# MeirBon/rendering-fw

Hardware: AMD Instinct MI355X
Metric: Msamples/sec at 1920x1080, 1M-tri scene; 1/2/4/8-GPU tile scaling (higher is better)
Workload: dtype f32; 1 GPU; terrain_1002k: 1002536 triangles, 1920x1080, pt integrator depth 2, 256 spp per step, 8 area-light triangles + 2 point lights, synthetic 2048x1024 HDR sky; parallelism=single GPU, no collective, streams=4, sample_group=64, csrc_hash=108fd956ff29d79e

## Files before the change

rendering-fw_amd/csrc/kernels.h:

```cpp
#pragma once
#include "rt_types.h"
#include <stddef.h>

namespace rtk
{

struct Params
{
	rt::SceneView sc;
	rt::WaveView wv;
	rt::CamView cam;
	rt::FrameView fr;
	uint32_t depth;
	uint32_t max_depth;
	uint32_t parity_no_jitter;
	uint32_t lds_first;
	uint32_t lds_count;
	uint32_t queue;
	uint32_t group;
	uint32_t refill;
	uint32_t textured;
};

enum GenMode
{
	GEN_BUFFER = 0,
	GEN_PT = 1,
	GEN_PARITY = 2,
	GEN_RANGED = 3
};

typedef void *stream_t;

struct DnView
{
	uint32_t W, H;
	rt::f4 *ga, *gb;
	rt::f4 *in, *out;
	rt::f4 *img[2];
	float *var[2];
	float sigma_l, sigma_n, sigma_z;
	uint32_t iterations;
	uint32_t *overflow;
	uint32_t *id;
	rt::f4 *hist;
};

struct DnTemporal
{
	rt::CamView cam, pcam;
	rt::FrameView fr;
	const rt::f4 *pgb;
	const uint32_t *id, *pid;
	const uint32_t *inst_ver;
	uint32_t n_inst, pscene;
	const rt::f4 *col_in;
	const float *mom_in, *n_in;
	float *mom_out, *n_out;
	float alpha;
	uint32_t usable;
};

constexpr uint32_t DN_M_INVALID = 0u, DN_M_STILL = 1u, DN_M_MOVED = 2u, DN_M_RESTART = 3u;
struct alignas(16) DnMotionInst
{
	float mp[12], mf[12];
	const rt::f4 *cur, *prev;
	const uint32_t *indices;
	uint32_t state, tri_count, vert_count, pad;
};
struct DnMotion
{
	const DnMotionInst *inst;
	const rt::f4 *surf;
// ... 117 lines not shown
```

rendering-fw_amd/csrc/kernels.hip:

```cpp
#include "kernels.h"
#include "rt_core.h"
#include "emu_streams.h"

#include <string.h>
#include <algorithm>

using namespace rt;

namespace rtk
{

constexpr int BLOCK = 256;
constexpr int KAT_IN = 24, KAT_OUT = 8;
#ifndef RT_TRAVERSAL_WAVES
#define RT_TRAVERSAL_WAVES 6
#endif
#ifndef RT_TRACE_WAVES
#define RT_TRACE_WAVES 8
#endif
#ifndef RT_TRACE_VGPRS
#define RT_TRACE_VGPRS 64
#endif
#ifndef RT_PRIMARY_WAVES
#define RT_PRIMARY_WAVES 7
// ... 65 lines not shown
	Ctx() { stk.lds = lds, stk.spill = spill, pot = potbuf, stk.top = nullptr, stk.top_first = 0, stk.top_count = 0, stk.overflow = &overflow_sink, stk.stride = 1; }
	explicit Ctx(const Params &p) : Ctx()
	{
		stk.overflow = &p.wv.counters->stack_overflow;
		stk.top = (const f4 *)(p.sc.nodes4 + p.lds_first), stk.top_first = p.lds_first, stk.top_count = p.lds_count;
	}
	struct OutQueue
	{
		uint32_t rays = 0;
	};
	OutQueue q_ext, q_shadow;
	uint32_t alloc(OutQueue &q, bool flag, uint32_t *queue_len)
	{
		if (!flag)
			return 0u;
		q.rays++;
		return (*queue_len)++;
	}
	void add64(unsigned long long *dst, uint32_t v) { *dst += v; }
};

#endif

RT_FN void primary_finish_item(const Params &q, uint32_t idx, f3 D, const Hit &h)
{
	int prim = h.prim;
	if (prim < 0)
	{
		f3 radiance = mk3(0, 0, 0);
		const f3 contribution = (mk3(1, 1, 1) * m_rcp(1.0f)) * pt_sky(q.sc, D);
		if (!any_nan(contribution))
			radiance = clamp_intensity(contribution, q.cam.clamp_value);
		q.wv.rad[idx] = mk4(radiance.x, radiance.y, radiance.z, q.wv.rad_nee ? -1.0f : 1.0f);
		prim = HIT_MISS_SHADED;
	}
	q.wv.hit0[idx] = mk4(h.t, h.u, h.v, ubits((uint32_t)prim));
	q.wv.hit0_inst[idx] = h.inst;
	if (prim >= 0)
	{
		float zero = 0.0f, one = 1.0f;
#if defined(__HIP_DEVICE_COMPILE__)
		asm volatile("" : "+v"(zero), "+v"(one));
#endif
		q.wv.rad[idx] = mk4(zero, zero, zero, one);
	}
}

template <int GEN, bool COUNT>
RT_FN void extend_item(const Params &p, uint32_t i, bool active, Ctx &ctx)
{
	f3 O = mk3(0, 0, 0), D = mk3(0, 0, 1);
	const uint32_t b = p.depth & 1u;
	float t_min = 1e-5f, t_max = 1e34f;
	if (GEN == GEN_BUFFER || GEN == GEN_RANGED)
	{
		if (active)
		{
			const f4 o4 = p.wv.org[b][i], d4 = p.wv.dir[b][i];
			O = xyz(o4), D = xyz(d4);
			if (GEN == GEN_RANGED)
				t_min = o4.w, t_max = d4.w;
			else if (fbits(o4.w) == RAY_VOID)
			{
				p.wv.hit[i] = mk4(0, 0, 0, ubits((uint32_t)HIT_VOID));
				active = false;
			}
		}
	}
	else
	{
		const PixelRef pr = slot_to_pixel(p.fr, i);
		active = active && pr.valid;
		if (GEN == GEN_PT)
		{
			if (active)
				pt_primary_ray(p.cam, p.fr, pr.x, pr.y, p.fr.sample_base + pr.sample, O, D);
		}
		else
		{
			const uint32_t npx = p.fr.W / 4u, npy = p.fr.H / 2u;
			active = active && pr.x < npx * 4u && pr.y < npy * 2u;
			if (active)
			{
				float r0 = 0.5f, r1 = 0.5f, r2 = 0.5f, r3 = 0.5f;
				if (!p.parity_no_jitter)
				{
					const uint32_t packet = (pr.y / 2u) * npx + pr.x / 4u;
					const uint32_t lane = (pr.y & 1u) * 4u + (pr.x & 3u);
					const uint32_t *sp = p.wv.packet_rng + 4ull * ((unsigned long long)pr.sample * npx * npy + packet);
					uint32_t s[4] = {sp[0], sp[1], sp[2], sp[3]};
					const bool lens = p.cam.aperture != 0.0f;
					const uint32_t draws = lens ? 32u : 16u;
					for (uint32_t k = 0; k < draws; k++)
					{
						const float r = u32_to_unit(xor128_next(s));
						if (k == lane)
							r0 = r;
						else if (k == 8u + lane)
							r1 = r;
						else if (k == 16u + lane)
							r2 = r;
						else if (k == 24u + lane)
							r3 = r;
					}
				}
				parity_primary_ray(p.cam, p.fr, pr.x, pr.y, r0, r1, r2, r3, O, D);
			}
		}
		if (active && GEN != GEN_PT)
		{
			p.wv.org[0][i] = mk4(O.x, O.y, O.z, ubits((i << 1) | 1u));
			p.wv.dir[0][i] = mk4(D.x, D.y, D.z, 0.0f);
		}
	}
	Hit h;
	h.t = 1e34f, h.u = 0, h.v = 0, h.prim = -1, h.inst = -1;
	TStat st;
	st.inner = 0, st.tris = 0, st.lds = 0;
	if (active)
	{
		trace<false, COUNT>(p.sc, O, D, t_min, t_max, h, ctx.stk, st);
		if (GEN == GEN_PT)
			primary_finish_item(p, i, D, h);
		else
		{
			f4 *hb = p.depth == 0 ? p.wv.hit0 : p.wv.hit;
			int *ib = p.depth == 0 ? p.wv.hit0_inst : p.wv.hit_inst;
			hb[i] = mk4(h.t, h.u, h.v, ubits((uint32_t)h.prim));
			ib[i] = h.inst;
		}
	}
	if (COUNT)
	{
		ctx.add64(&p.wv.counters->inner_extend, st.inner);
		ctx.add64(&p.wv.counters->tris_extend, st.tris);
		ctx.add64(&p.wv.counters->lds_extend, st.lds);
		ctx.add64(&p.wv.counters->rays_extend, active ? 1u : 0u);
	}
}

template <bool COUNT>
RT_FN void shade_parity_item(const Params &p, uint32_t i, bool active, Ctx &ctx)
{
	const PixelRef pr = slot_to_pixel(p.fr, i);
	active = active && pr.valid && pr.x < (p.fr.W / 4u) * 4u && pr.y < (p.fr.H / 2u) * 2u;
	TStat st;
	st.inner = 0, st.tris = 0, st.lds = 0;
	uint32_t nshadow = 0;
	f4 out = mk4(0, 0, 0, 0);
	if (active)
	{
		const f4 o4 = p.wv.org[0][i], d4 = p.wv.dir[0][i], h4 = p.wv.hit0[i];
		Hit h;
		h.t = h4.x, h.u = h4.y, h.v = h4.z, h.prim = (int)fbits(h4.w), h.inst = p.wv.hit0_inst[i];
		if (h.prim < 0)
		{
			const f3 s = parity_sky(p.sc, xyz(d4));
			out = mk4(s.x, s.y, s.z, 0.0f);
		}
		else
		{
			if (pr.sample == 0 && pr.y * p.fr.W + pr.x == p.fr.probe_pixel)
			{
				WaveCounters *c = p.wv.counters;
				c->probe_inst = (uint32_t)h.inst, c->probe_prim = (uint32_t)h.prim, c->probe_dist = h.t, c->probe_valid = 1u;
			}
			out = parity_shade<COUNT>(p.sc, xyz(o4), xyz(d4), h, ctx.stk, st, nshadow);
		}
	}
	if (pr.valid)
		p.wv.rad[i] = out;
	if (COUNT)
	{
		ctx.add64(&p.wv.counters->inner_shadow, st.inner);
		ctx.add64(&p.wv.counters->tris_shadow, st.tris);
		ctx.add64(&p.wv.counters->lds_shadow, st.lds);
		ctx.add64(&p.wv.counters->rays_shadow, nshadow);
		ctx.add64(&p.wv.counters->shaded, (active && out.w > 0.0f) ? 1u : 0u);
	}
}

#if defined(RT_DIAG_SHADE_CLOCK)
__device__ unsigned long long g_shade_clk[32];
#define RT_ITEM_CLK , ClkProbe *clk
#define RT_ITEM_TICK(K) clk_tick(*clk, K)
#else
#define RT_ITEM_CLK
#define RT_ITEM_TICK(K)
#endif
struct ShadeSink
{
	const Params &p;
	Ctx &ctx;
	uint32_t slot;
	RT_FN void probe(const Hit &h) const
	{
		WaveCounters *c = p.wv.counters;
		c->probe_inst = (uint32_t)h.inst, c->probe_prim = (uint32_t)h.prim, c->probe_dist = h.t, c->probe_valid = 1u;
	}
	RT_FN void shadow(bool emit, const f4 &so, const f4 &sd, const f4 &se)
	{
		const uint32_t si = ctx.alloc(ctx.q_shadow, emit, &p.wv.counters->shadow_n[p.depth]);
		if (emit)
		{
			p.wv.sh_org[si] = so;
			p.wv.sh_dir[si] = sd;
			if (p.depth != 0 || !p.wv.rad_nee)
				p.wv.sh_rad[si] = se;
			else
				p.wv.rad_nee[slot] = mk4(0.0f + se.x, 0.0f + se.y, 0.0f + se.z, 0.0f);
		}
	}
};

template <bool TEX, bool SKY, bool LT> RT_FN void shade_pt_item(const Params &p, const SkyView &sky, const LightTreeView &lt, uint32_t i, bool active, const f4 &h4, int hi, Ctx &ctx RT_ITEM_CLK)
{
	RT_ITEM_TICK(0);
	const uint32_t b = p.depth & 1u, nb = b ^ 1u;
	ShadeOut out;
	PathIn in;
	in.O = mk3(0, 0, 0), in.D = mk3(0, 0, 1), in.T = mk3(1, 1, 1), in.bsdfPdf = 1.0f;
	in.slot = 0, in.flags = 0, in.packedN = 0, in.depth = p.depth;
	Hit h;
	h.t = h4.x, h.u = h4.y, h.v = h4.z, h.prim = (int)fbits(h4.w), h.inst = hi;
	if (active && p.depth == 0)
	{
		const PixelRef pr = slot_to_pixel(p.fr, i);
		pt_primary_ray(p.cam, p.fr, pr.x, pr.y, p.fr.sample_base + pr.sample, in.O, in.D);
		in.slot = i, in.flags = 1u, in.packedN = 0u;
	}
	else if (active)
	{
		const f4 o4 = (p.depth == 0 && p.cam.aperture == 0.0f) ? mk4(p.cam.pos.x, p.cam.pos.y, p.cam.pos.z, ubits((i << 1) | 1u)) : p.wv.org[b][i];
		const f4 d4 = p.wv.dir[b][i];
		in.O = xyz(o4), in.D = xyz(d4);
		const uint32_t ow = fbits(o4.w);
		in.slot = ow >> 1, in.flags = ow & 1u, in.packedN = fbits(d4.w);
		if (p.depth != 0)
		{
			const f4 t4 = p.wv.thr[b][i];
			in.T = xyz(t4), in.bsdfPdf = t4.w;
		}
	}
	const uint32_t slot = in.slot;
	ShadeSink sink{p, ctx, slot};
	pt_shade<TEX, SKY, LT>(p.sc, sky, lt, p.cam, p.fr, p.max_depth, active, in, h, out, ctx.pot, sink RT_CLK_ARG);
	if (active)
	{
		if (p.depth == 0)
		{
			const bool ends = p.wv.rad_nee && !out.emit_shadow && !out.emit_ext;
			if (h.prim < 0 || ends || out.radiance.x != 0.0f || out.radiance.y != 0.0f || out.radiance.z != 0.0f)
				p.wv.rad[slot] = mk4(out.radiance.x, out.radiance.y, out.radiance.z, ends ? -1.0f : 1.0f);
			if (p.wv.rad_nee && out.emit_ext && !out.emit_shadow)
				p.wv.rad_nee[slot] = mk4(0, 0, 0, 0);
		}
		else if (out.radiance.x != 0.0f || out.radiance.y != 0.0f || out.radiance.z != 0.0f)
		{
			f4 r = p.wv.rad[slot];
			r.x += out.radiance.x, r.y += out.radiance.y, r.z += out.radiance.z;
			p.wv.rad[slot] = r;
		}
	}
	RT_ITEM_TICK(7);
	const uint32_t ei = ctx.alloc(ctx.q_ext, out.emit_ext, &p.wv.counters->ext_n[p.depth + 1]);
	if (out.emit_ext)
	{
		p.wv.org[nb][ei] = out.eo;
		p.wv.dir[nb][ei] = out.ed;
		p.wv.thr[nb][ei] = out.et;
	}
	RT_ITEM_TICK(8);
}

RT_FN void connect_finish(const Params &p, uint32_t i, uint32_t slot, bool visible)
{
	if (p.depth == 0 && p.wv.rad_nee)
	{
		if (!visible)
			p.wv.rad_nee[slot] = mk4(0, 0, 0, 0);
	}
	else if (visible)
	{
		const f4 e4 = p.wv.sh_rad[i];
		f4 *const dst = p.wv.rad_nee ? p.wv.rad_nee : p.wv.rad;
		f4 r = dst[slot];
		r.x += e4.x, r.y += e4.y, r.z += e4.z;
		dst[slot] = r;
	}
}
RT_FN uint32_t shadow_slot(const Params &p, uint32_t word)
{
	return (p.depth == 0 && p.fr.shadow_bins) ? word & ((1u << shadow_slot_bits(p.fr.shadow_bins)) - 1u) : word;
}
RT_FN void connect_skip_item(const Params &p, uint32_t i)
// ... 655 lines not shown
			const uint32_t base = q_next;
			const uint32_t take = nidle < q_end - q_next ? nidle : q_end - q_next;
			q_next += take;
			const uint32_t limit = base + take;
			if (!has_ray)
			{
				const uint32_t idx = base + wave_prefix(idle_mask);
				if (idx < limit)
				{
					{
						typedef float v4f_ __attribute__((ext_vector_type(4)));
						v4f_ oa = *(const v4f_ *)(ray_o + idx), da = *(const v4f_ *)(ray_d + idx);
						asm volatile("" : "+v"(oa), "+v"(da));
						const f4 o4 = mk4(oa.x, oa.y, oa.z, oa.w), d4 = mk4(da.x, da.y, da.z, da.w);
						if (fbits(o4.w) == RAY_VOID)
						{
							if (!ANY)
								p.wv.hit[idx] = mk4(0, 0, 0, ubits((uint32_t)HIT_VOID));
						}
						else
						{
							T.begin(p.sc, xyz(o4), xyz(d4), 1e-5f, ANY ? d4.w : 1e34f);
							has_ray = true, ray = idx, slot = ANY ? shadow_slot(p, fbits(o4.w)) : fbits(o4.w), nrays++;
						}
					}
				}
			}
			exhausted = q_next >= count;
		}
		if (__ballot(has_ray) == 0ull)
		{
			if (exhausted)
				break;
			continue;
		}
		RT_TRACE_TICK(0)
		T.template descend<VOTE>(p.sc, ctx.stk, st);
		RT_TRACE_TICK(1)
		const auto world = [&](f3 &O, f3 &D) {
			const f4 o4 = ray_o[ray], d4 = ray_d[ray];
			O = xyz(o4), D = xyz(d4);
		};
		if (has_ray)
			T.visit(p.sc, ctx.stk, st, world);
		RT_TRACE_TICK(2)
		if (has_ray)
		{
			if (T.done())
			{
				if (ANY)
					connect_finish(p, ray, slot, T.hit.prim < 0);
				else
				{
					p.wv.hit[ray] = mk4(T.hit.t, T.hit.u, T.hit.v, ubits((uint32_t)T.hit.prim));
					p.wv.hit_inst[ray] = T.hit.inst;
				}
				has_ray = false;
			}
		}
		RT_TRACE_TICK(3)
	}
#if defined(RT_DIAG_TRACE_CLOCK)
	if (lane == 0u)
		for (int k = 0; k < 4; k++)
			atomicAdd(&g_trace_clk[MODE == STREAM_ANY ? 1 : 0][k], clk_acc[k]), atomicAdd(&g_trace_clk[MODE == STREAM_ANY ? 1 : 0][4 + k], clk_n[k]);
#endif
	if (COUNT)
	{
		ctx.add64(ANY ? &wc->inner_shadow : &wc->inner_extend, st.inner);
		ctx.add64(ANY ? &wc->tris_shadow : &wc->tris_extend, st.tris);
		ctx.add64(ANY ? &wc->lds_shadow : &wc->lds_extend, st.lds);
		ctx.add64(ANY ? &wc->rays_shadow : &wc->rays_extend, nrays);
	}
}

template <bool ANY, bool COUNT>
__global__ void __launch_bounds__(TRACE_BLOCK, ANY ? RT_ANY_WAVES : RT_TRACE_WAVES) __attribute__((amdgpu_num_vgpr(RT_TRACE_VGPRS))) k_trace_stream(const Params p)
{
	const uint32_t count = ANY ? connection_count(p.wv.counters, p.depth) : p.wv.counters->ext_n[p.depth];
	if (count == 0u)
	{
		if (ANY && p.depth == 0 && p.wv.rad_nee)
			for (uint32_t i = blockIdx.x * TRACE_BLOCK + threadIdx.x, n = p.wv.counters->shadow_n[0]; i < n; i += gridDim.x * TRACE_BLOCK)
				connect_skip_item(p, i);
		return;
	}
	if (!ANY)
		clock_in(p.wv.counters, p.depth);
	RT_STACK_DECL_N(ANY ? LDS_STACK_ANY : LDS_STACK, TRACE_BLOCK)
	stream_rays<ANY ? STREAM_ANY : STREAM_EXT, COUNT>(p, count, ctx);
	if (!ANY)
		clock_out(p.wv.counters, p.depth);
}

template <bool COUNT>
__global__ void __launch_bounds__(TRACE_BLOCK, RT_TRACE_WAVES) __attribute__((amdgpu_num_vgpr(RT_TRACE_VGPRS))) k_trace_fused(const Params pe, const Params pa)
{
	const uint32_t count_e = pe.wv.counters->ext_n[pe.depth];
	const uint32_t count_a = connection_count(pa.wv.counters, pa.depth);
	if (count_a == 0u && pa.depth == 0 && pa.wv.rad_nee)
		for (uint32_t i = blockIdx.x * TRACE_BLOCK + threadIdx.x, n = pa.wv.counters->shadow_n[0]; i < n; i += gridDim.x * TRACE_BLOCK)
			connect_skip_item(pa, i);
	if (count_e == 0u && count_a == 0u)
		return;
	const Params &p = pe;
	RT_STACK_DECL_N(LDS_STACK, TRACE_BLOCK)
	const unsigned long long t0 = threadIdx.x == 0 ? (unsigned long long)wall_clock64() : 0ull;
	if (count_e)
// ... 1214 lines not shown
```

rendering-fw_amd/csrc/rfwhip_api.cpp:

```cpp
#include "rfwhip.h"

#include "bvh_build.h"
#include "device_layer.h"
#include "internal.h"
#include "kernels.h"
#include "rt_types.h"
#include "sky_sampling.h"
#include "light_tree.h"

#include <algorithm>
#include <chrono>
#include <cmath>
#include <cstdarg>
#include <cstdio>
#include <cstdlib>
#include <cstring>
#include <string>
#include <vector>

using rt::f4;

static thread_local char g_error[1024] = "";
int rfwhip_internal_set_error(int code, const char *fmt, ...)
{
// ... 237 lines not shown
	int dn_temporal = 0;
	float dn_alpha = 0.2f;
	DevBuf d_dn_prev, d_dn_ids, d_dn_hist, d_dn_inst_ver;
	unsigned long long frame_serial = 0;
	unsigned long long samples_total = 0;
	uint32_t sample_origin = 0;
	bool dn_have_pres = false;
	unsigned long long dn_pres_serial = 0;
	rt::CamView dn_pres_cam{};
	uint32_t dn_pres_scene = 0, dn_pres_W = 0, dn_pres_H = 0;
	bool dn_guides_pres = false;
	bool dn_prev_ok = false;
	unsigned long long dn_saved_serial = 0;
	bool dn_reset_since = false;
	int dn_hist_cur = 0;
	bool dn_t_usable = false;
	rt::CamView dn_t_pcam{};
	uint32_t dn_t_pscene = 0;
	std::vector<uint32_t> dn_inst_ver;
	bool dn_inst_ver_stale = true;
	int dn_motion = 0;
	DevBuf d_dn_surf, d_dn_minst;
	std::vector<DnInstSnap> dn_g_rec, dn_p_rec;
	bool dn_g_rec_ok = false, dn_p_rec_ok = false;
	unsigned long long dn_pres_id = 1;
	unsigned long long dn_edit_count = 0;
	std::vector<rtk::DnMotionInst> dn_mtab;
	uint32_t dn_mtab_scene = 0;
	unsigned long long dn_mtab_edits = 0;
	bool dn_mtab_stale = true;

	std::vector<MeshRec> meshes;
	std::vector<InstRec> instances;
	rfwhip_light_count lc = {0, 0, 0, 0};
	bool scene_dirty = true;

	DevBuf d_nodes4f;
	bool nodes4f_current = false;
	size_t nodes4_live = 0;
	DevBuf d_nodes, d_nodes4, d_nodes4_src, d_tri_verts, d_tri_shade, d_tri_uv, d_tlas_prims, d_instances;
	size_t blas_nodes4 = 0, node4_capacity = 0;
	DevBuf d_materials, d_textures, d_tex_u32, d_tex_f4, d_sky, d_area, d_point, d_spot, d_dir;
	uint32_t material_count = 0, texture_count = 0, sky_w = 0, sky_h = 0;
	bool textured = false;
	int sky_sampling = 0;
	float sky_pick = -1.0f;
	uint64_t sky_version = 0;
	uint64_t sky_table_of = ~0ull;
	double sky_total = 0.0;
	DevBuf d_sky_alias;
	rt::SkyView sky_view{};
	bool sky_stale = false;
	int light_sampling = 0;
	int display_tonemap = 0, display_fxaa = 1, display_srgb = 0;
	DevBuf d_display;
	int noise_estimate = 0;
	float noise_floor = 0.01f, noise_threshold = 0.05f;
	bool noise_live = false;
	DevBuf d_noise, d_noise_map, d_noise_tiles, d_noise_total, d_noise_in;
	int adaptive_sampling = 0, adaptive_min_samples = 16, adaptive_every = 4;
	bool adaptive_live = false;
	uint32_t adaptive_calls = 0;
	DevBuf d_ad_n, d_ad_active, d_ad_mask;
	dm::event_t ev_adaptive;
	bool adaptive_mask_moved = false;
	uint64_t adaptive_serial = 0, adaptive_seen[MAX_SUB] = {};
	DevBuf d_lt_nodes, d_lt_paths;
	rt::LightTreeView lt_view{};
	bool lt_stale = false;
	uint32_t tlas_root_entry = 0, instance_count = 0;
	rt::SceneView sv;

	DevBuf d_org[2], d_dir2[2], d_thr[2], d_hit, d_hit_inst, d_hit0, d_hit0_inst, d_hit0_done, d_sh_org[2], d_sh_dir[2], d_sh_rad[2],
		d_rad[2], d_rad_nee[2], d_acc, d_counters, d_packet_rng, d_jump_table, d_present;
	uint32_t samples_done = 0;
	size_t wave_capacity = 0;
	size_t rad_capacity[2] = {0, 0};
	rt::FrameView fr;
	bool jump_table_uploaded = false;

	uint32_t rng_state[4] = {123456789u, 362436069u, 521288629u, 88675123u};
	std::vector<uint32_t> jump_table;

	uint32_t probe_x = 0, probe_y = 0;
	uint32_t probe_inst = 0, probe_prim = 0;
	float probe_dist = 0;

	std::vector<TimedSpan> spans;
	std::vector<dm::event_t> event_pool;
	size_t events_used = 0;
	float kernel_ms[KF_COUNT] = {0, 0, 0, 0, 0, 0, 0, 0, 0};
	uint32_t kernel_launches[KF_COUNT] = {0, 0, 0, 0, 0, 0, 0, 0, 0};
	rfwhip_render_stats stats;
	std::chrono::steady_clock::time_point render_t0;
	bool render_pending = false;
	rfwhip_counters totals;
};

static void mat4_inverse(const float *m, float *inv)
{
	float t[16];
	t[0] = m[5] * m[10] * m[15] - m[5] * m[11] * m[14] - m[9] * m[6] * m[15] + m[9] * m[7] * m[14] + m[13] * m[6] * m[11] - m[13] * m[7] * m[10];
	t[4] = -m[4] * m[10] * m[15] + m[4] * m[11] * m[14] + m[8] * m[6] * m[15] - m[8] * m[7] * m[14] - m[12] * m[6] * m[11] + m[12] * m[7] * m[10];
	t[8] = m[4] * m[9] * m[15] - m[4] * m[11] * m[13] - m[8] * m[5] * m[15] + m[8] * m[7] * m[13] + m[12] * m[5] * m[11] - m[12] * m[7] * m[9];
	t[12] = -m[4] * m[9] * m[14] + m[4] * m[10] * m[13] + m[8] * m[5] * m[14] - m[8] * m[6] * m[13] - m[12] * m[5] * m[10] + m[12] * m[6] * m[9];
	t[1] = -m[1] * m[10] * m[15] + m[1] * m[11] * m[14] + m[9] * m[2] * m[15] - m[9] * m[3] * m[14] - m[13] * m[2] * m[11] + m[13] * m[3] * m[10];
// ... 1484 lines not shown
	}
};

static void fill_params(rfwhip_context *c, const rfwhip_camera *cam, rtk::Params &p)
{
	memset(&p, 0, sizeof(p));
	p.sc = c->sv;
	rt::WaveView &wv = p.wv;
	for (int k = 0; k < 2; k++)
		wv.org[k] = c->d_org[k].as<f4>(), wv.dir[k] = c->d_dir2[k].as<f4>(), wv.thr[k] = c->d_thr[k].as<f4>();
	wv.hit = c->d_hit.as<f4>(), wv.hit_inst = c->d_hit_inst.as<int>();
	wv.hit0 = c->d_hit0.as<f4>(), wv.hit0_inst = c->d_hit0_inst.as<int>(), wv.hit0_done = nullptr;
	wv.sh_org = c->d_sh_org[0].as<f4>(), wv.sh_dir = c->d_sh_dir[0].as<f4>(), wv.sh_rad = c->d_sh_rad[0].as<f4>();
	wv.rad = c->d_rad[0].as<f4>(), wv.rad_nee = nullptr, wv.acc = c->d_acc.as<f4>();
	wv.packet_rng = c->d_packet_rng.as<uint32_t>();
	wv.counters = c->d_counters.as<rt::WaveCounters>();
	p.cam.blue_noise = nullptr;
	if (cam)
	{
		rfwhip_camera_view v;
		rfwhip_camera_get_view(cam, &v);
		p.cam.pos = rt::f3{v.pos[0], v.pos[1], v.pos[2]};
		p.cam.p1 = rt::f3{v.p1[0], v.p1[1], v.p1[2]};
		p.cam.right = rt::f3{v.p2[0] - v.p1[0], v.p2[1] - v.p1[1], v.p2[2] - v.p1[2]};
		p.cam.up = rt::f3{v.p3[0] - v.p1[0], v.p3[1] - v.p1[1], v.p3[2] - v.p1[2]};
		p.cam.aperture = v.aperture, p.cam.spread_angle = v.spreadAngle, p.cam.clamp_value = cam->clampValue;
		p.cam.blue_noise = (c->sampler == 1 && c->have_blue_noise) ? c->d_blue_noise.as<uint32_t>() : nullptr;
	}
	p.fr = c->fr;
	p.fr.spp = (uint32_t)c->spp;
	p.fr.sample_base = c->sample_origin + c->samples_done;
	p.fr.probe_pixel = c->probe_y * c->W + c->probe_x;
	p.max_depth = (uint32_t)c->max_depth;
	p.parity_no_jitter = c->jitter == 1;
	p.lds_first = 0, p.lds_count = 0;
	{
		uint32_t big_base = 0, big_count = 0;
		for (size_t mi = 0; mi < c->meshes.size(); mi++)
		{
			const MeshRec &m = c->meshes[mi];
			const bool in_world = c->wtree.valid && mi < c->wtree.mesh_all.size() && c->wtree.mesh_all[mi];
			if (m.used && !in_world && m.n4_count > big_count)
				big_base = (uint32_t)m.n4_base, big_count = m.n4_count;
		}
		if (c->wtree.valid && c->wtree.resident && c->wtree.n4.size() > big_count)
			big_base = c->wtree.n4_base, big_count = (uint32_t)c->wtree.n4.size();
		const uint32_t cap = rtk::max_lds_nodes();
		const uint32_t want = c->lds_nodes < 0 ? cap : std::min<uint32_t>((uint32_t)c->lds_nodes, cap);
		if (big_count && want)
			p.lds_first = big_base, p.lds_count = std::min<uint32_t>(want, big_count);
	}
	p.refill = (uint32_t)c->refill & ((c->packet_ok && c->nodes4f_current) ? 15u : 7u);
	p.textured = c->textured ? 1u : 0u;
}

static int sync_all(rfwhip_context *c)
{
	for (int i = 0; i < rfwhip_context::MAX_SUB; i++)
	{
		if (c->sub_stream[i])
			RF_TRY(dm::sync(c->sub_stream[i]));
		if (c->conn_stream[i])
			RF_TRY(dm::sync(c->conn_stream[i]));
	}
	RF_TRY(dm::sync(c->stream));
	if (c->present_pending)
	{
		RF_TRY(dm::event_sync(c->ev_present_out));
		c->present_pending = false;
	}
	if (c->dn_pending)
	{
		RF_TRY(dm::event_sync(c->ev_dn));
		c->dn_pending = false;
	}
	return 0;
}

static int ensure_sub_batches(rfwhip_context *c, int subs)
{
	if (!c->events_ready)
	{
		RF_TRY(dm::event_create(&c->ev_prologue));
		for (int r = 0; r < rfwhip_context::MAX_RING; r++)
			RF_TRY(dm::event_create(&c->ev_resolve[r]));
		RF_TRY(dm::event_create(&c->ev_present_in));
		RF_TRY(dm::event_create(&c->ev_present_out));
		RF_TRY(dm::event_create(&c->ev_dn));
		RF_TRY(dm::event_create(&c->ev_adaptive));
		for (int i = 0; i < rfwhip_context::MAX_SUB; i++)
		{
			RF_TRY(dm::event_create(&c->ev_sub_done[i]));
			RF_TRY(dm::event_create(&c->ev_conn_last[i]));
			for (int d = 0; d < rt::MAX_DEPTH_SLOTS; d++)
			{
				RF_TRY(dm::event_create(&c->ev_shade[i][d]));
				RF_TRY(dm::event_create(&c->ev_conn[i][d]));
			}
		}
		c->events_ready = true;
	}
	for (int i = 0; i < subs; i++)
	{
		if (!c->sub_stream[i])
			RF_TRY(dm::stream_create(&c->sub_stream[i]));
		if (!c->conn_stream[i])
// ... 187 lines not shown
		if (c->adaptive_live && c->adaptive_seen[i] != c->adaptive_serial)
		{
			RF_TRY(dm::stream_wait_event(s, c->ev_adaptive));
			c->adaptive_seen[i] = c->adaptive_serial;
		}
		rtk::Params p = base;
		const size_t off_rad = (size_t)c->fr.slots * s_begin;
		const size_t off = alternate ? (paths + pad) * par : off_rad + (size_t)k * pad;
		for (int q = 0; q < 2; q++)
			p.wv.org[q] += off, p.wv.dir[q] += off, p.wv.thr[q] += off;
		p.wv.hit += off, p.wv.hit_inst += off, p.wv.hit0 += off, p.wv.hit0_inst += off;
		p.wv.rad += off_rad;
		if (p.wv.rad_nee)
			p.wv.rad_nee += off_rad;
		if (p.wv.packet_rng)
			p.wv.packet_rng += (size_t)s_begin * packets * 4;
		if (i > 0)
			p.wv.counters = c->d_counters_sub[i].as<rt::WaveCounters>();
		p.fr.spp = spp_i;
		p.fr.sample_base = c->sample_origin + c->samples_done + s_begin;
		const uint32_t n = c->fr.slots * spp_i;
		p.fr.shadow_bins = 0u;
		if (c->integrator == 1 && connect && (c->shadow_packets > 0 || (c->shadow_packets < 0 && c->shadow_packets_auto_on)) && (p.refill & 8u) &&
			sgroup_log2 >= 3u && !side)
			for (uint32_t b = rt::SHADOW_BIN_BITS; b >= 1u && !p.fr.shadow_bins; b--)
				if ((unsigned long long)n <= (1ull << rt::shadow_slot_bits(b)))
					p.fr.shadow_bins = b;
		p.wv.hit0_done = c->integrator == 1 && c->group_flags && rtk::primary_packet_form(p, n) && (size_t)i < HIT0_DONE_PAD / 2
							 ? c->d_hit0_done.as<unsigned char>() + (off >> 6) + (size_t)i
							 : nullptr;
		rtk::launch_init_counters(p.wv.counters, n, s);
		uint32_t queue = 0;
		bool conn_now = false;
		bool sp_side_pending = false;
		if (c->integrator == 0)
		{
			p.depth = 0, p.group = row_group, p.queue = queue++;
			StageTimer te(c, KF_EXTEND, 0, s);
			rtk::launch_extend(p, rtk::GEN_PARITY, count, n, s);
			te.stop();
			p.queue = queue++;
			StageTimer ts(c, KF_SHADE, -1, s);
			rtk::launch_shade_parity(p, count, n, s);
			ts.stop();
		}
		else
		{
			rtk::Params pa = p;
			bool pa_pending = false;
			for (int d = 0; d <= c->max_depth; d++)
			{
				p.depth = (uint32_t)d;
				p.group = d == 0 ? row_group : 16u;
				p.queue = queue++;
				p.wv.sh_org = c->d_sh_org[d & 1].as<f4>() + off, p.wv.sh_dir = c->d_sh_dir[d & 1].as<f4>() + off;
				p.wv.sh_rad = c->d_sh_rad[d & 1].as<f4>() + off;
				StageTimer te(c, KF_EXTEND, d, s);
				const uint32_t n_ext = depth_items(c, n, d, false), n_shade = depth_items(c, n, d, true);
				te.fused = pa_pending;
				if (pa_pending && sp_side_pending)
				{
					RF_TRY(dm::stream_wait_event(s, c->ev_conn[i][0]));
					sp_side_pending = false;
				}
				if (pa_pending)
					rtk::launch_trace_fused(p, pa, count, n_ext, s);
				else if (d == 0 && c->adaptive_live)
					rtk::launch_extend_masked(p, ad.mask, count, n, s);
				else
					rtk::launch_extend(p, d == 0 ? rtk::GEN_PT : rtk::GEN_BUFFER, count, d == 0 ? n : n_ext, s);
				pa_pending = false;
				te.stop();
				if (side && d >= 2 && d < c->max_depth)
					RF_TRY(dm::stream_wait_event(s, c->ev_conn[i][d - 2]));
				StageTimer ts(c, KF_SHADE, -1, s);
				if (c->light_sampling)
					rtk::launch_shade_pt_lt(p, c->sky_view, c->lt_view, n_shade, s);
				else
					rtk::launch_shade_pt(p, c->sky_view, n_shade, s);
				ts.stop();
				if (c->adaptive_live && connect && d < c->max_depth)
					rtk::launch_adaptive_connections(p.wv.counters, (uint32_t)d, s);
				if (connect && d < c->max_depth)
				{
					if (d == 0 && p.fr.shadow_bins)
					{
						p.group = 16u, p.queue = queue++;
						void *const sp_stream = c->shadow_side ? c->conn_stream[i] : s;
						if (c->shadow_side)
						{
							RF_TRY(dm::event_record(c->ev_shade[i][0], s));
							RF_TRY(dm::stream_wait_event(sp_stream, c->ev_shade[i][0]));
						}
						StageTimer tc(c, KF_CONNECT, -1, sp_stream);
						rtk::launch_shadow_packets(p, count, depth_items(c, n, 1, false), sp_stream);
						tc.stop();
						if (c->shadow_side)
						{
							RF_TRY(dm::event_record(c->ev_conn[i][0], sp_stream));
							sp_side_pending = true;
						}
						continue;
					}
					if (fused)
					{
						pa = p, pa.group = 16u, pa.queue = queue++;
// ... 1126 lines not shown
	{"shadow_packets_on", nullptr, GET { return put(out, cap, "%d", (c->shadow_packets > 0 || (c->shadow_packets < 0 && c->shadow_packets_auto_on)) && c->packet_ok && c->nodes4f_current && (c->refill & 8) ? 1 : 0); }, false},
	{"shadow_bins_per_run", nullptr, GET { return put(out, cap, "%.3f", c->shadow_bins_per_run); }, false},
	{"textured", nullptr, GET { return put(out, cap, "%d", c->textured ? 1 : 0); }, false},
	{"packet", nullptr, GET { return put(out, cap, "%d", (c->packet_ok && (c->refill & 8)) ? 1 : 0); }, false},
	{"world_tree", nullptr, GET { return put(out, cap, "%zu", c->wtree.valid ? c->wtree.tris : (size_t)0); }, false},
	{"light_sampling", SET {
		 static const char *const names[] = {"reference", "linear", "tree"};
		 int mode = -1;
		 for (int k = 0; k < 3; k++)
			 if (!strcmp(value, names[k]))
				 mode = k;
		 if (mode < 0)
			 return set_error(RFWHIP_ERR_INVALID_ARGUMENT, "%s must be \"reference\", \"linear\" or \"tree\"", key);
		 c->light_sampling = mode;
		 c->lt_stale = true;
		 return RFWHIP_OK; },
	 GET { return put(out, cap, "%s", c->light_sampling == 2 ? "tree" : c->light_sampling == 1 ? "linear" : "reference"); }, false},
	{"display_tonemap", ENUM2(display_tonemap, "aces", "none"), false},
	{"display_fxaa", SET {
		 bool on;
		 RF_TRY(parse_01(key, value, &on));
		 c->display_fxaa = on;
		 return RFWHIP_OK; },
	 GET_INT(display_fxaa), false},
	{"display_srgb", SET {
		 bool on;
		 RF_TRY(parse_01(key, value, &on));
		 c->display_srgb = on;
		 return RFWHIP_OK; },
	 GET_INT(display_srgb), false},
	{"noise_estimate", SET {
		 bool on;
		 RF_TRY(parse_01(key, value, &on));
		 if (!on && (c->adaptive_sampling || c->adaptive_live))
			 return set_error(RFWHIP_ERR_STATE, c->adaptive_sampling ? "noise_estimate: adaptive_sampling is on and needs it; turn that off first"
																	 : "noise_estimate: the accumulation is an adaptive one; render with RFWHIP_RESET first");
		 if (!on && c->noise_estimate)
		 {
			 RF_TRY(sync_all(c));
			 c->d_noise.free_(), c->d_noise_map.free_(), c->d_noise_tiles.free_(), c->d_noise_total.free_();
			 c->noise_live = false;
		 }
		 c->noise_estimate = on;
		 return RFWHIP_OK; },
	 GET_INT(noise_estimate), false},
	{"adaptive_sampling", SET {
		 bool on;
		 RF_TRY(parse_01(key, value, &on));
		 if (on && !c->noise_estimate)
			 return set_error(RFWHIP_ERR_STATE, "adaptive_sampling needs noise_estimate=1");
		 c->adaptive_sampling = on;
		 return RFWHIP_OK; },
	 GET_INT(adaptive_sampling), false},
	{"adaptive_min_samples", SET { return set_int_in(c->adaptive_min_samples, key, value, 2, 1 << 30); }, GET_INT(adaptive_min_samples), false},
	{"adaptive_every", SET { return set_int_in(c->adaptive_every, key, value, 1, 64); }, GET_INT(adaptive_every), false},
	{"noise_floor", SET { return set_float(c->noise_floor, key, value, [](float f) { return f > 0.0f && f < 1e30f; }, "be a finite number > 0", false); },
	 GET { return put(out, cap, "%g", c->noise_floor); }, false},
	{"noise_threshold", SET { return set_float(c->noise_threshold, key, value, [](float f) { return f > 0.0f && f < 1e30f; }, "be a finite number > 0", false); },
	 GET { return put(out, cap, "%g", c->noise_threshold); }, false},
	{"light_tree", nullptr, GET {
		 if (c->lt_stale)
			 RF_TRY(update_light_tree(c));
		 return put(out, cap, "%u", c->lt_view.node_count); },
	 false},
	{"sky", nullptr, GET {
		 if (c->sky_stale && !c->scene_dirty)
			 RF_TRY(update_sky_sampling(c));
		 return put(out, cap, "%d", c->sky_view.pick > 0.0f ? 1 : 0); },
	 false},
};
#undef SET
#undef GET
#undef GET_INT
#undef ENUM2
#undef FLAG
#undef INT_IN
#undef SIGMA

static const Setting *find_setting(const char *key)
{
	for (const Setting &s : k_settings)
		if (!strcmp(s.key, key))
			return &s;
	return nullptr;
}

extern "C" int rfwhip_set_setting(rfwhip_context *c, const char *key, const char *value)
{
	CTX_ENTER(c);
	if (!key || !value)
		return set_error(RFWHIP_ERR_INVALID_ARGUMENT, "null key/value");
	const Setting *s = find_setting(key);
	if (!s || !s->set)
		return set_error(RFWHIP_ERR_INVALID_ARGUMENT, "unknown setting \"%s\"", key);
	return s->set(c, key, value);
}

extern "C" int rfwhip_get_setting(rfwhip_context *c, const char *key, char *value, size_t cap)
{
	CTX_ENTER(c);
	if (!key || !value || !cap)
		return set_error(RFWHIP_ERR_INVALID_ARGUMENT, "null key/value");
	const Setting *s = find_setting(key);
	if (!s)
		return set_error(RFWHIP_ERR_INVALID_ARGUMENT, "unknown setting \"%s\"", key);
	return s->get(c, value, cap);
// ... 687 lines not shown
	}
	RF_TRY(sync_all(c));
	const size_t n4 = std::min<size_t>(node_cap, m.n4_count), nt = std::min<size_t>(tri_cap, m.triCount);
	if (nodes4c && n4)
		RF_TRY(dm::d2h(nodes4c, c->d_nodes4.as<rt::Node4c>() + m.n4_base, n4 * sizeof(rt::Node4c), c->stream));
	if (src4 && n4)
		RF_TRY(dm::d2h(src4, c->d_nodes4_src.as<uint32_t>() + 4ull * m.n4_base, 4 * n4 * sizeof(uint32_t), c->stream));
	if (tri_verts && nt)
		RF_TRY(dm::d2h(tri_verts, c->d_tri_verts.as<f4>() + 3ull * m.tri_base, 3 * nt * sizeof(f4), c->stream));
	if (nodes4f && n4)
	{
		if (c->nodes4f_current)
			RF_TRY(dm::d2h(nodes4f, c->d_nodes4f.as<rt::Node4f>() + m.n4_base, n4 * sizeof(rt::Node4f), c->stream));
		else
		{
			DevBuf tmp;
			int rc = tmp.ensure(n4 * sizeof(rt::Node4f));
			if (!rc)
			{
				rtk::launch_expand4(c->d_nodes4.as<rt::Node4c>() + m.n4_base, tmp.as<rt::Node4f>(), (uint32_t)n4, c->stream);
				rc = dm::last_launch_error();
			}
			if (!rc)
				rc = dm::d2h(nodes4f, tmp.p, n4 * sizeof(rt::Node4f), c->stream);
			tmp.free_();
			RF_TRY(rc);
		}
	}
	return RFWHIP_OK;
}

#if defined(RFWHIP_HOST_EMULATION) && defined(RFWHIP_EMU_STREAMS) && RFWHIP_EMU_STREAMS
extern "C" RFWHIP_API int rfwhip_emu_set_schedule(int policy, unsigned seed)
{
	if (policy < emu_streams::INORDER || policy > emu_streams::EAGER)
		return set_error(RFWHIP_ERR_INVALID_ARGUMENT, "rfwhip_emu_set_schedule: unknown policy %d", policy);
	emu_streams::state().policy = emu_streams::INORDER;
	emu_streams::set_schedule(policy, seed);
	return RFWHIP_OK;
}
extern "C" RFWHIP_API int rfwhip_emu_schedule_stats(unsigned long long *ran, unsigned long long *out_of_order,
												   unsigned long long *shadow_packet_launches)
{
	const emu_streams::State &S = emu_streams::state();
	if (ran)
		*ran = S.ran;
	if (out_of_order)
		*out_of_order = S.out_of_order;
	if (shadow_packet_launches)
		*shadow_packet_launches = S.shadow_packet_launches;
	return RFWHIP_OK;
}
#endif
```

rendering-fw_amd/csrc/shade_pt_body.h:

```cpp
	static_assert(BLOCK == POT_STRIDE, "potential cache layout is pot[light][thread]");
	__shared__ float s_pot[POT_SLOTS * BLOCK];
	Ctx ctx;
	ctx.stk.lds = nullptr, ctx.stk.spill = nullptr, ctx.stk.top = nullptr, ctx.stk.top_first = 0, ctx.stk.top_count = 0;
	ctx.stk.overflow = nullptr, ctx.stk.stride = 0;
	ctx.pot = s_pot + threadIdx.x;
	const uint32_t count = p.wv.counters->ext_n[p.depth];
	constexpr uint32_t QN = 128u, QM = QN - 1u;
	__shared__ f4 s_qhit[BLOCK / 64][QN];
	__shared__ uint32_t s_qidx[BLOCK / 64][QN];
	__shared__ int s_qinst[BLOCK / 64][QN];
	__shared__ uint32_t s_qmiss[BLOCK / 64][QN];
	const uint32_t lane = threadIdx.x & 63u, wave = (uint32_t)__builtin_amdgcn_readfirstlane((int)(threadIdx.x >> 6));
	f4 *const qhit = s_qhit[wave];
	uint32_t *const qidx = s_qidx[wave], *const qmiss = s_qmiss[wave];
	int *const qinst = s_qinst[wave];
	const f4 *const hits = p.depth == 0 ? p.wv.hit0 : p.wv.hit;
	const int *const insts = p.depth == 0 ? p.wv.hit0_inst : p.wv.hit_inst;
	const uint32_t nchunks = (count + 63u) / 64u;
	const uint32_t nwaves = gridDim.x * (BLOCK / 64u);
	{
		const uint32_t per_wave = count / (nwaves * 4u);
		ctx.q_block = per_wave > QUEUE_BLOCK ? QUEUE_BLOCK : (per_wave < 64u ? 0u : per_wave);
	}
#if defined(RT_DIAG_SHADE_CLOCK)
	__shared__ unsigned long long s_clk[BLOCK / 64][32];
	if (lane < 32u)
		s_clk[wave][lane] = 0ull;
	ClkProbe clk;
	clk.last = __builtin_readcyclecounter(), clk.acc = s_clk[wave];
#endif
#ifndef RT_SHADE_RUN
#define RT_SHADE_RUN 32u
#endif
	uint32_t srun = nchunks / (nwaves * 4u);
	srun = srun > RT_SHADE_RUN ? RT_SHADE_RUN : (srun ? srun : 1u);
	uint32_t c = (blockIdx.x * (BLOCK / 64u) + wave) * srun;
	uint32_t c_left = srun;
	uint32_t hq = 0, nq = 0;
	uint32_t mq = 0, nm = 0;
	uint32_t nshaded = 0;
	static_assert(RT_SHADE_RUN <= 32u, "run_done is a 32-bit mask");
	const unsigned char *const done = p.depth == 0 ? p.wv.hit0_done : nullptr;
	uint32_t run_done = 0;
#pragma nounroll
	for (;;)
	{
		uint32_t idx = 0;
		bool act = false;
		f4 h4 = mk4(0, 0, 0, ubits((uint32_t)-1));
		int hi = -1;
		const bool drain = c >= nchunks;
		const bool take_hits = nq >= 64u || (drain && nq > 0u);
		if (take_hits)
		{
			const uint32_t n = nq < 64u ? nq : 64u, e = (hq + lane) & QM;
			nshaded += n;
			act = lane < n;
			idx = qidx[e], h4 = qhit[e], hi = qinst[e];
			hq = (hq + n) & QM, nq -= n;
		}
		else if (nm >= 64u || (drain && nm > 0u))
		{
			const uint32_t n = nm < 64u ? nm : 64u;
			act = lane < n;
			idx = qmiss[(mq + lane) & QM];
			mq = (mq + n) & QM, nm -= n;
		}
		else if (!drain)
		{
			if (done && c_left == srun)
				run_done = (uint32_t)__ballot(lane < srun && c + lane < nchunks && done[c + lane] != 0);
			const bool skip = (run_done >> (srun - c_left)) & 1u;
			idx = c * 64u + lane;
			if (--c_left)
				c++;
			else
				c += (nwaves - 1u) * srun + 1u, c_left = srun;
			if (skip)
				continue;
			bool valid = idx < count;
			if (p.depth == 0 && valid)
				valid = slot_to_pixel(p.fr, idx).valid;
			if (valid)
				h4 = hits[idx], hi = insts[idx];
			const int prim = valid ? (int)fbits(h4.w) : HIT_VOID;
			const bool is_hit = prim >= 0;
			const unsigned long long m = __ballot(is_hit);
			if (is_hit)
			{
				const uint32_t e = (hq + nq + wave_prefix(m)) & QM;
				qidx[e] = idx, qhit[e] = h4, qinst[e] = hi;
			}
			nq += (uint32_t)__popcll(m);
			const bool is_miss = prim == -1;
			const unsigned long long mm = __ballot(is_miss);
			if (is_miss)
				qmiss[(mq + nm + wave_prefix(mm)) & QM] = idx;
			nm += (uint32_t)__popcll(mm);
#if defined(RT_DIAG_SHADE_CLOCK)
			clk_tick(clk, 14);
#endif
			continue;
		}
		else
			break;
		__builtin_amdgcn_wave_barrier();
#if defined(RT_DIAG_SHADE_CLOCK)
		shade_pt_item<TEX, SKY, LT>(p, sky, lt, idx, act, h4, hi, ctx, &clk);
#else
		shade_pt_item<TEX, SKY, LT>(fresh_params(), sky, lt, idx, act, h4, hi, ctx);
#endif
	}
#if defined(RT_DIAG_SHADE_CLOCK)
	if (lane < 32u)
		atomicAdd(g_shade_clk + lane, s_clk[wave][lane]);
#endif
	WaveCounters *const wc = p.wv.counters;
	const uint32_t nb = (p.depth & 1u) ^ 1u;
	for (uint32_t s = ctx.q_ext.pos + lane; s < ctx.q_ext.end; s += 64u)
// ... 13 lines not shown
```

Baseline: 5782 Msamples/s.

## Store miss direction and slot in hit records to skip origin/dir reloads

At depth one and beyond, rays that miss now write their direction and packed slot word into the hit and hit-instance buffers instead of t/u/v and instance. When shading a miss, the shader reads the direction and slot from that record plus throughput, and no longer loads the origin and direction buffers. This cuts scattered memory reads for sky-miss shading. The cost is extra logic in trace and shade, the shade miss queue now reloading the hit record, and an unconditional throughput load on the normal path. A test readback API and a runtime toggle, on by default, are also added.

```diff
diff --git a/rendering-fw_amd/csrc/kernels.h b/rendering-fw_amd/csrc/kernels.h
--- a/rendering-fw_amd/csrc/kernels.h
+++ b/rendering-fw_amd/csrc/kernels.h
@@ -20,6 +20,7 @@
 	uint32_t group;
 	uint32_t refill;
 	uint32_t textured;
+	uint32_t miss_records;
 };
 
 enum GenMode
diff --git a/rendering-fw_amd/csrc/kernels.hip b/rendering-fw_amd/csrc/kernels.hip
--- a/rendering-fw_amd/csrc/kernels.hip
+++ b/rendering-fw_amd/csrc/kernels.hip
@@ -141,12 +141,14 @@
 	f3 O = mk3(0, 0, 0), D = mk3(0, 0, 1);
 	const uint32_t b = p.depth & 1u;
 	float t_min = 1e-5f, t_max = 1e34f;
+	uint32_t slot_word = 0u;
 	if (GEN == GEN_BUFFER || GEN == GEN_RANGED)
 	{
 		if (active)
 		{
 			const f4 o4 = p.wv.org[b][i], d4 = p.wv.dir[b][i];
 			O = xyz(o4), D = xyz(d4);
+			slot_word = fbits(o4.w);
 			if (GEN == GEN_RANGED)
 				t_min = o4.w, t_max = d4.w;
 			else if (fbits(o4.w) == RAY_VOID)
@@ -215,8 +217,9 @@
 		{
 			f4 *hb = p.depth == 0 ? p.wv.hit0 : p.wv.hit;
 			int *ib = p.depth == 0 ? p.wv.hit0_inst : p.wv.hit_inst;
-			hb[i] = mk4(h.t, h.u, h.v, ubits((uint32_t)h.prim));
-			ib[i] = h.inst;
+			const bool miss_rec = GEN == GEN_BUFFER && p.miss_records && h.prim < 0;
+			hb[i] = miss_rec ? mk4(D.x, D.y, D.z, ubits((uint32_t)-1)) : mk4(h.t, h.u, h.v, ubits((uint32_t)h.prim));
+			ib[i] = miss_rec ? (int)slot_word : h.inst;
 		}
 	}
 	if (COUNT)
@@ -318,18 +321,23 @@
 		pt_primary_ray(p.cam, p.fr, pr.x, pr.y, p.fr.sample_base + pr.sample, in.O, in.D);
 		in.slot = i, in.flags = 1u, in.packedN = 0u;
 	}
+	else if (active && p.miss_records && h.prim == -1)
+	{
+		in.D = mk3(h4.x, h4.y, h4.z);
+		const uint32_t ow = (uint32_t)hi;
+		in.slot = ow >> 1, in.flags = ow & 1u;
+		const f4 t4 = p.wv.thr[b][i];
+		in.T = xyz(t4), in.bsdfPdf = t4.w;
+	}
 	else if (active)
 	{
-		const f4 o4 = (p.depth == 0 && p.cam.aperture == 0.0f) ? mk4(p.cam.pos.x, p.cam.pos.y, p.cam.pos.z, ubits((i << 1) | 1u)) : p.wv.org[b][i];
+		const f4 o4 = p.wv.org[b][i];
 		const f4 d4 = p.wv.dir[b][i];
 		in.O = xyz(o4), in.D = xyz(d4);
 		const uint32_t ow = fbits(o4.w);
 		in.slot = ow >> 1, in.flags = ow & 1u, in.packedN = fbits(d4.w);
-		if (p.depth != 0)
-		{
-			const f4 t4 = p.wv.thr[b][i];
-			in.T = xyz(t4), in.bsdfPdf = t4.w;
-		}
+		const f4 t4 = p.wv.thr[b][i];
+		in.T = xyz(t4), in.bsdfPdf = t4.w;
 	}
 	const uint32_t slot = in.slot;
 	ShadeSink sink{p, ctx, slot};
@@ -1091,8 +1099,16 @@
 					connect_finish(p, ray, slot, T.hit.prim < 0);
 				else
 				{
-					p.wv.hit[ray] = mk4(T.hit.t, T.hit.u, T.hit.v, ubits((uint32_t)T.hit.prim));
-					p.wv.hit_inst[ray] = T.hit.inst;
+					if (p.miss_records && T.hit.prim < 0)
+					{
+						p.wv.hit[ray] = mk4(T.d.x, T.d.y, T.d.z, ubits((uint32_t)-1));
+						p.wv.hit_inst[ray] = (int)slot;
+					}
+					else
+					{
+						p.wv.hit[ray] = mk4(T.hit.t, T.hit.u, T.hit.v, ubits((uint32_t)T.hit.prim));
+						p.wv.hit_inst[ray] = T.hit.inst;
+					}
 				}
 				has_ray = false;
 			}
diff --git a/rendering-fw_amd/csrc/rfwhip_api.cpp b/rendering-fw_amd/csrc/rfwhip_api.cpp
--- a/rendering-fw_amd/csrc/rfwhip_api.cpp
+++ b/rendering-fw_amd/csrc/rfwhip_api.cpp
@@ -313,6 +313,7 @@
 	rt::SkyView sky_view{};
 	bool sky_stale = false;
 	int light_sampling = 0;
+	int miss_records = 1;
 	int display_tonemap = 0, display_fxaa = 1, display_srgb = 0;
 	DevBuf d_display;
 	int noise_estimate = 0;
@@ -1903,6 +1904,7 @@
 	}
 	p.refill = (uint32_t)c->refill & ((c->packet_ok && c->nodes4f_current) ? 15u : 7u);
 	p.textured = c->textured ? 1u : 0u;
+	p.miss_records = 0u;
 }
 
 static int sync_all(rfwhip_context *c)
@@ -2196,6 +2198,7 @@
 			{
 				p.depth = (uint32_t)d;
 				p.group = d == 0 ? row_group : 16u;
+				p.miss_records = d >= 1 && c->miss_records ? 1u : 0u;
 				p.queue = queue++;
 				p.wv.sh_org = c->d_sh_org[d & 1].as<f4>() + off, p.wv.sh_dir = c->d_sh_dir[d & 1].as<f4>() + off;
 				p.wv.sh_rad = c->d_sh_rad[d & 1].as<f4>() + off;
@@ -3428,6 +3431,12 @@
 		 c->adaptive_sampling = on;
 		 return RFWHIP_OK; },
 	 GET_INT(adaptive_sampling), false},
+	{"miss_records", SET {
+		 bool on;
+		 RF_TRY(parse_01(key, value, &on));
+		 c->miss_records = on;
+		 return RFWHIP_OK; },
+	 GET_INT(miss_records), false},
 	{"adaptive_min_samples", SET { return set_int_in(c->adaptive_min_samples, key, value, 2, 1 << 30); }, GET_INT(adaptive_min_samples), false},
 	{"adaptive_every", SET { return set_int_in(c->adaptive_every, key, value, 1, 64); }, GET_INT(adaptive_every), false},
 	{"noise_floor", SET { return set_float(c->noise_floor, key, value, [](float f) { return f > 0.0f && f < 1e30f; }, "be a finite number > 0", false); },
@@ -4221,3 +4230,28 @@
 	return RFWHIP_OK;
 }
 #endif
+
+extern "C" RFWHIP_API int rfwhip_test_read_wave(rfwhip_context *c, unsigned depth, size_t cap, float *org, float *dir, float *hit, int *hit_inst,
+												 unsigned *count)
+{
+	CTX_ENTER(c);
+	if (depth < 1u || depth >= (unsigned)rt::MAX_DEPTH_SLOTS)
+		return set_error(RFWHIP_ERR_INVALID_ARGUMENT, "rfwhip_test_read_wave: depth %u", depth);
+	RF_TRY(sync_all(c));
+	rt::WaveCounters wc;
+	RF_TRY(dm::d2h(&wc, c->subs_first == 0 ? c->d_counters.p : c->d_counters_sub[c->subs_first].p, sizeof(wc), c->stream));
+	const size_t n = std::min((size_t)wc.ext_n[depth], cap), off = c->last_wave_off;
+	if ((off + n) * sizeof(f4) > c->d_hit.cap || (off + n) * sizeof(f4) > c->d_org[depth & 1u].cap)
+		return set_error(RFWHIP_ERR_STATE, "rfwhip_test_read_wave: no wave of that size was rendered");
+	if (count)
+		*count = wc.ext_n[depth];
+	if (n && org)
+		RF_TRY(dm::d2h(org, c->d_org[depth & 1u].as<f4>() + off, n * sizeof(f4), c->stream));
+	if (n && dir)
+		RF_TRY(dm::d2h(dir, c->d_dir2[depth & 1u].as<f4>() + off, n * sizeof(f4), c->stream));
+	if (n && hit)
+		RF_TRY(dm::d2h(hit, c->d_hit.as<f4>() + off, n * sizeof(f4), c->stream));
+	if (n && hit_inst)
+		RF_TRY(dm::d2h(hit_inst, c->d_hit_inst.as<int>() + off, n * 4, c->stream));
+	return RFWHIP_OK;
+}
diff --git a/rendering-fw_amd/csrc/shade_pt_body.h b/rendering-fw_amd/csrc/shade_pt_body.h
--- a/rendering-fw_amd/csrc/shade_pt_body.h
+++ b/rendering-fw_amd/csrc/shade_pt_body.h
@@ -65,6 +65,8 @@
 			act = lane < n;
 			idx = qmiss[(mq + lane) & QM];
 			mq = (mq + n) & QM, nm -= n;
+			if (p.miss_records && act)
+				h4 = hits[idx], hi = insts[idx];
 		}
 		else if (!drain)
 		{
```

Measured after the change: 5842 Msamples/s, median of 4. 1.1% higher.
